# Owen1B/KAIR

Hardware: AMD Instinct MI355X
Metric: train patches/sec + PSNR, SwinIR x4 48-px LQ, at 1/2/4/8 MI355X (higher is better)
Workload: dtype fp32x3

## Files before the change

### kair_amd/csrc/gemm_x3.hip

```cpp
#include <string.h>

#include <type_traits>

#include "gemm_common.h"

namespace {

template <typename T> struct RawX3 { Raw<T> h, l; };

KAIR_DEV f32x4 mfma16(const f16x8& a, const f16x8& b, f32x4 c) {
  return __builtin_amdgcn_mfma_f32_16x16x32_f16(a, b, c, 0, 0, 0);
}

KAIR_DEV void commit_lo_plane(f16* dst, const Raw<f16>& raw, const Pend& pd) {
  f16x8 q = __builtin_bit_cast(f16x8, raw.a);
  if (pd.scale == 0.f) q = f16x8{};
  if (pd.ones >= 0) q[pd.ones] = (f16)0.f;
  *(f16x8*)dst = q;
}

template <typename T>
KAIR_DEV void commit_pair(f16* hi, f16* lo, const RawX3<T>& raw, const Pend& pd, float onev) {
  if constexpr (sizeof(T) == 4) {
    commit_chunk<f16, T>(hi, raw.h, pd, false, onev);
// ... 34 lines not shown
  const int n0 = tn * BN;
  const int tid = threadIdx.x, lane = tid & 63, wave = tid >> 6;
  const int wm = wave / WN, wn = wave % WN;
  const int KB = 2 * ((K + 63) / 64) * 64;

  RowState ra[PA], rb[PB];
#pragma unroll
  for (int p = 0; p < PA; ++p) {
    const int c = tid + p * NT;
    ra[p] = row_state<AM, TA>(A, c < CA ? m0 + c / CPR : A.M);
    ra[p].scale *= A.x3s;
  }
#pragma unroll
  for (int p = 0; p < PB; ++p) {
    const int c = tid + p * NT;
    rb[p] = row_state<AM_ROWS, f16>(B, c < CB ? (long)(n0 + c / CPR) : B.M);
  }
  RawX3<TA> va[PA];
  Raw<f16> vbh[PB], vbl[PB];
  Pend pa[PA], pb[PB], pbl[PB];
  auto gload = [&](int kt) {
    const int k0 = kt * BK;
#pragma unroll
    for (int p = 0; p < PA; ++p) {
      const int k = k0 + ((tid + p * NT) % CPR) * 8;
      issue_chunk<AM, TA>(A, ra[p], k, K, va[p].h, pa[p]);
      if constexpr (sizeof(TA) == 2) {
        Pend d;
        issue_chunk<AM, TA>(A, ra[p], k, K, va[p].l, d, A.lo_ptr);
      }
    }
    const int kb = (k0 >> 6) * 128 + (k0 & 63);
#pragma unroll
    for (int p = 0; p < PB; ++p) {
      const int k = kb + ((tid + p * NT) % CPR) * 8;
      issue_chunk<AM_ROWS, f16>(B, rb[p], k, KB, vbh[p], pb[p]);
      issue_chunk<AM_ROWS, f16>(B, rb[p], k + 64, KB, vbl[p], pbl[p]);
    }
  };
  auto sstore = [&](int st) {
    f16* s0 = lds + st * STAGE;
#pragma unroll
    for (int p = 0; p < PA; ++p) {
      const int c = tid + p * NT;
      if (c < CA) {
        const int o = (c / CPR) * LD + (c % CPR) * 8;
        commit_pair<TA>(s0 + o, s0 + PLANE + o, va[p], pa[p], 1.f);
      }
    }
#pragma unroll
    for (int p = 0; p < PB; ++p) {
      const int c = tid + p * NT;
      if (c < CB) {
        const int o = BM * LD + (c / CPR) * LD + (c % CPR) * 8;
        commit_chunk<f16, f16>(s0 + o, vbh[p], pb[p]);
        commit_chunk<f16, f16>(s0 + PLANE + o, vbl[p], pbl[p]);
      }
    }
  };

  f32x4 acc[RM][RN];
#pragma unroll
  for (int i = 0; i < RM; ++i)
#pragma unroll
    for (int j = 0; j < RN; ++j) acc[i][j] = f32x4{0.f, 0.f, 0.f, 0.f};

  const int fr = lane & 15, fq = lane >> 4;
  const int nk = (K + BK - 1) / BK;
  gload(0);
  sstore(0);
  __syncthreads();
  for (int kt = 0; kt < nk; ++kt) {
    const int st = kt & 1;
    if (kt + 1 < nk) gload(kt + 1);
    const f16* sAh = lds + st * STAGE;
    const f16* sBh = sAh + BM * LD;
    const f16* sAl = sAh + PLANE;
    const f16* sBl = sAl + BM * LD;
    f16x8 ah[RM], al[RM], bh[RN], bl[RN];
#pragma unroll
    for (int i = 0; i < RM; ++i) {
      const int o = (wm * TM + i * 16 + fr) * LD + fq * 8;
      ah[i] = *(const f16x8*)(sAh + o);
      al[i] = *(const f16x8*)(sAl + o);
    }
#pragma unroll
    for (int j = 0; j < RN; ++j) {
      const int o = (wn * TN + j * 16 + fr) * LD + fq * 8;
      bh[j] = *(const f16x8*)(sBh + o);
      bl[j] = *(const f16x8*)(sBl + o);
    }
#pragma unroll
    for (int i = 0; i < RM; ++i)
#pragma unroll
      for (int j = 0; j < RN; ++j) {
        acc[i][j] = mfma16(ah[i], bh[j], acc[i][j]);
        acc[i][j] = mfma16(ah[i], bl[j], acc[i][j]);
        acc[i][j] = mfma16(al[i], bh[j], acc[i][j]);
      }
    if (kt + 1 < nk) sstore(st ^ 1);
    __syncthreads();
  }
  float* et = (float*)smem;
#pragma unroll
  for (int i = 0; i < RM; ++i)
#pragma unroll
    for (int j = 0; j < RN; ++j)
#pragma unroll
      for (int r = 0; r < 4; ++r) et[(wm * TM + i * 16 + fq * 4 + r) * EPI_LD + wn * TN + j * 16 + fr] = acc[i][j][r];
  __syncthreads();
  constexpr int CH = BM * BN / 8;
  for (int c = tid; c < CH; c += NT) {
    const int row = c / (BN / 8), col = (c % (BN / 8)) * 8;
    float v[8];
    const float4 a = *(const float4*)(et + row * EPI_LD + col);
    const float4 b = *(const float4*)(et + row * EPI_LD + col + 4);
    v[0] = a.x; v[1] = a.y; v[2] = a.z; v[3] = a.w; v[4] = b.x; v[5] = b.y; v[6] = b.z; v[7] = b.w;
#pragma unroll
    for (int j = 0; j < 8; ++j) v[j] *= E.acc_scale;
    epi_chunk(E, m0 + row, n0 + col, v);
  }
}

template <typename TA, typename TB, int AMB, int BN, int BKo>
__global__ __launch_bounds__(NT, 2) void gemm_tn_x3_kernel(Op A, Op B, float* ws, long M, int N, int K, long rows_per_split,
                                                           int tilesK, float acc_scale) {
  constexpr int BMr = 32;
  constexpr int LDA = BN + 8, LDB = BKo + 8;
  constexpr int WN = 2, WK = 2;
  constexpr int TN_ = BN / WN, TK_ = BKo / WK;
  constexpr int RN = TN_ / 16, RK = TK_ / 16;
  constexpr int CPA = BN / 8, CPB = BKo / 8;
  constexpr int CA = BMr * CPA, CB = BMr * CPB;
  constexpr int PA = (CA + NT - 1) / NT, PB = (CB + NT - 1) / NT;
  constexpr int PL = BMr * (LDA + LDB);
  constexpr int STAGE = 2 * PL;
  __shared__ __attribute__((aligned(16))) f16 lds[2 * STAGE];

  const int tn = blockIdx.x / tilesK, tk = blockIdx.x - (blockIdx.x / tilesK) * tilesK;
  const int n0 = tn * BN, k0 = tk * BKo;
  const long mbeg = (long)blockIdx.y * rows_per_split;
  long mend = mbeg + rows_per_split;
  if (mend > M) mend = M;
  const int tid = threadIdx.x, lane = tid & 63, wave = tid >> 6;
  const int wn = wave / WK, wk = wave % WK;

  RawX3<TA> va[PA];
  RawX3<TB> vb[PB];
  Pend pa[PA], pb[PB];
  auto gload = [&](long mb) {
#pragma unroll
    for (int p = 0; p < PA; ++p) {
      const int c = tid + p * NT;
      if (c < CA) {
        const long m = mb + c / CPA;
        RowState r = row_state<AM_ROWS, TA>(A, m < mend ? m : A.M);
        r.scale *= A.x3s;
        issue_chunk<AM_ROWS, TA>(A, r, n0 + (c % CPA) * 8, N, va[p].h, pa[p]);
        if constexpr (sizeof(TA) == 2) {
          Pend d;
          issue_chunk<AM_ROWS, TA>(A, r, n0 + (c % CPA) * 8, N, va[p].l, d, A.lo_ptr);
        }
      }
    }
#pragma unroll
    for (int p = 0; p < PB; ++p) {
      const int c = tid + p * NT;
      if (c < CB) {
        const long m = mb + c / CPB;
        RowState r = row_state<AMB, TB>(B, m < mend ? m : B.M);
        r.scale *= B.x3s;
        issue_chunk<AMB, TB>(B, r, k0 + (c % CPB) * 8, K, vb[p].h, pb[p]);
        if constexpr (sizeof(TB) == 2) {
          Pend d;
          issue_chunk<AMB, TB>(B, r, k0 + (c % CPB) * 8, K, vb[p].l, d, B.lo_ptr);
        }
      }
    }
  };
  const float onea = ldexpf(1.f, A.x3_exp), oneb = ldexpf(1.f, B.x3_exp);
  auto sstore = [&](int st) {
    f16* sAh = lds + st * STAGE;
    f16* sBh = sAh + BMr * LDA;
#pragma unroll
    for (int p = 0; p < PA; ++p) {
      const int c = tid + p * NT;
      if (c < CA) {
        const int o = (c / CPA) * LDA + (c % CPA) * 8;
        commit_pair<TA>(sAh + o, sAh + PL + o, va[p], pa[p], onea);
      }
    }
#pragma unroll
    for (int p = 0; p < PB; ++p) {
      const int c = tid + p * NT;
      if (c < CB) {
        const int o = (c / CPB) * LDB + (c % CPB) * 8;
        commit_pair<TB>(sBh + o, sBh + PL + o, vb[p], pb[p], oneb);
      }
    }
  };

  f32x4 acc[RN][RK];
#pragma unroll
  for (int i = 0; i < RN; ++i)
#pragma unroll
    for (int j = 0; j < RK; ++j) acc[i][j] = f32x4{0.f, 0.f, 0.f, 0.f};

  const int nsteps = mbeg < mend ? (int)((mend - mbeg + BMr - 1) / BMr) : 0;
  if (nsteps > 0) {
    gload(mbeg);
    sstore(0);
    __syncthreads();
  }
  const int q = (lane & 15) >> 2, p4 = (lane & 3) * 4, g8 = (lane >> 4) * 8;
  for (int it = 0; it < nsteps; ++it) {
    const int st = it & 1;
    if (it + 1 < nsteps) gload(mbeg + (long)(it + 1) * BMr);
    const f16* sAh = lds + st * STAGE;
    const f16* sBh = sAh + BMr * LDA;
    const f16* sAl = sAh + PL;
    const f16* sBl = sBh + PL;
    f16x8 ah[RN], al[RN], bh[RK], bl[RK];
#pragma unroll
    for (int i = 0; i < RN; ++i) {
      const int o = (g8 + q) * LDA + wn * TN_ + i * 16 + p4;
      ah[i] = trfrag<f16>(sAh + o, LDA);
      al[i] = trfrag<f16>(sAl + o, LDA);
    }
#pragma unroll
    for (int j = 0; j < RK; ++j) {
      const int o = (g8 + q) * LDB + wk * TK_ + j * 16 + p4;
      bh[j] = trfrag<f16>(sBh + o, LDB);
      bl[j] = trfrag<f16>(sBl + o, LDB);
    }
#pragma unroll
    for (int i = 0; i < RN; ++i)
#pragma unroll
      for (int j = 0; j < RK; ++j) {
        acc[i][j] = mfma16(ah[i], bh[j], acc[i][j]);
        acc[i][j] = mfma16(ah[i], bl[j], acc[i][j]);
        acc[i][j] = mfma16(al[i], bh[j], acc[i][j]);
      }
    if (it + 1 < nsteps) sstore(st ^ 1);
    __syncthreads();
  }
  const int fr = lane & 15, fq = lane >> 4;
  float* P = ws + (long)blockIdx.y * N * K;
#pragma unroll
  for (int i = 0; i < RN; ++i)
#pragma unroll
    for (int j = 0; j < RK; ++j)
#pragma unroll
      for (int r = 0; r < 4; ++r) {
        const int n = n0 + wn * TN_ + i * 16 + fq * 4 + r;
        const int k = k0 + wk * TK_ + j * 16 + fr;
        if (n < N && k < K) P[(long)n * K + k] = acc[i][j][r] * acc_scale;
      }
}

constexpr int XR_BM = 128, XR_NB = 3, XR_ASTAGE = XR_BM * 128;
template <int BN> struct XR {
  static constexpr int BSTAGE = BN * 128, NA = BN <= 192 ? 5 : 4, LDS = NA * XR_ASTAGE + XR_NB * BSTAGE + BN * 4;
  static constexpr int RN = BN / 32;
  static constexpr int BI = BN / 64;
};

enum { XE_ROWS_F32 = 0, XE_ROWS_PAIR = 1, XE_QKV = 2, XE_PSHUF = 3, XE_PUNSHUF = 4 };

constexpr int XS_CTAS = 4, XS_IT = 64, XS_N = 5;
__device__ unsigned long long g_x3_stamps[XS_CTAS * 8 * XS_IT * XS_N];
KAIR_DEV unsigned long long x3_now() {
  unsigned long long t;
  asm volatile("s_memtime %0\n\ts_waitcnt lgkmcnt(0)" : "=s"(t)::"memory");
  return t;
}

enum { XA_NONE = 0, XA_GELU = 1, XA_GELU_X = 2, XA_LEAKY = 3 };
enum { XG_MUL = 4, XG_LEAKY = 2 };

template <typename TA, int AM, int EM, int EX, int ACT, int GK, int BN, int BM = XR_BM>
__global__ __launch_bounds__(512, 1) void gemm_nt_x3_ring(Op A, Op B, Epi E, int K, int tilesN, int tilesM, int m_base) {
  constexpr int NA = XR<BN>::NA, RN = XR<BN>::RN, NP = RN / 2, BI = XR<BN>::BI, BSTAGE = XR<BN>::BSTAGE, WC = BN / 2;
  constexpr int RI = BM / 64, ASTAGE = BM * 128;
  static_assert(RI == 1 || RI == 2, "64- or 128-row tiles");
  constexpr int XLDS = EX == EX_LNB ? (4 * 2 * 32 * 2 + 8) * 4 : 0;
  __shared__ __attribute__((aligned(16))) char smem[NA * ASTAGE + XR_NB * BSTAGE + BN * 4 + XLDS];
  char* const sA = smem;
  char* const sB = smem + NA * ASTAGE;
  float* const sBias = (float*)(sB + XR_NB * BSTAGE);
  const int tid = threadIdx.x, lane = tid & 63, wave = __builtin_amdgcn_readfirstlane(tid >> 6);
  const int grp = wave >> 2, wm = (wave >> 1) & 1, wn = wave & 1;
  const int fr = lane & 15, fq = lane >> 4, q8 = lane & 7;
  const int cta = xcd_remap(blockIdx.x, gridDim.x);
  const int nt = cta % tilesN, mstride = gridDim.x / tilesN, mt0 = cta / tilesN;
  if (mt0 >= tilesM) return;
  const int ntile = (tilesM - mt0 + mstride - 1) / mstride;
  const int nk = K / 32;
  const int total = ntile * nk;
  const int n0 = nt * BN;
  const f16* zero = (const f16*)g_kair_zero_line;

  constexpr bool SW = EM != XE_ROWS_F32;
  constexpr int CB = SW ? 4 : 16;
  int c8[NP], oc[NP];
  long colo[NP];
#pragma unroll
  for (int p = 0; p < NP; ++p) {
    const int n = SW ? n0 + wn * WC + (2 * p + (fq & 1)) * 16 + (fq >> 1) * 8 : n0 + wn * WC + 2 * p * 16 + 4 * fq;
    c8[p] = n;
    oc[p] = E.ones_col >= n + CB && E.ones_col < n + CB + 4 ? 4 + E.ones_col - n - CB
                                                            : (E.ones_col >= n && E.ones_col < n + 4 ? E.ones_col - n : -1);
    if constexpr (EM == XE_QKV) {
      const int pw = E.nh * E.hdp;
      const int part = fdiv(n, E.d_pw), rr = n - part * pw;
      const int h = fdiv(rr, E.d_hdp), d = rr - h * E.hdp;
      colo[p] = (long)part * E.M * pw + (long)h * E.tok * E.hdp + d;
    } else if constexpr (EM == XE_PSHUF) {
      const int nf = E.N / (E.r * E.r), sp = n / nf, c = n - sp * nf, i = sp / E.r, j = sp - i * E.r;
      colo[p] = ((long)i * E.psW * E.r + j) * E.ldo + c;
    } else {
      colo[p] = n;
    }
  }
  for (int i = tid; i < BN; i += 512) sBias[i] = E.bias && n0 + i < (EX == EX_LNB ? E.lnC : E.N) ? E.bias[n0 + i] : 0.f;
  if constexpr (EX == EX_LNB)
    if (tid < 8) ((int*)(sBias + BN + 4 * 2 * 32 * 2))[tid] = 0;
  const f16* bsrc[BI];
#pragma unroll
  for (int ii = 0; ii < BI; ++ii) {
    const int r = (wave * BI + ii) * 8 + (lane >> 3), u = q8 ^ (r & 7);
    bsrc[ii] = n0 + r < (int)B.M ? (const f16*)B.ptr + (long)(n0 + r) * B.ld + (u < 4 ? u * 8 : 64 + (u - 4) * 8) : nullptr;
  }
  long aoff[RI];
  int ay[RI], ax[RI], au[RI];
  bool aok[RI];
  auto load_rows = [&](int i) __attribute__((always_inline)) {
    const int mt = mt0 + i * mstride;
#pragma unroll
    for (int ii = 0; ii < RI; ++ii) {
      const int r = (wave * RI + ii) * 8 + (lane >> 3);
      const int m = m_base + mt * BM + r;
      au[ii] = q8 ^ (r & 7);
      aok[ii] = m < (int)A.M;
      const int mm = aok[ii] ? m : 0;
      if constexpr (AM == AM_ROWS) {
        aoff[ii] = (long)win_to_token32(mm, A.win) * A.ld;
      } else {
        const int hw = A.d_hw.d;
        const int b = fdiv(mm, A.d_hw), p = mm - b * hw;
        ay[ii] = fdiv(p, A.d_imW);
        ax[ii] = p - ay[ii] * A.imW;
        aoff[ii] = (long)b * (hw >> (2 * A.up_sh));
      }
    }
  };
  int at = 0, ak = 0, as_ = 0, bk = 0, bs = 0;
  int a_tap = 0, a_c0 = 0;
  const float* arow[RI];
#pragma unroll
  for (int ii = 0; ii < RI; ++ii) arow[ii] = nullptr;
  auto set_tap = [&]() __attribute__((always_inline)) {
    int dy = a_tap / 3 - 1, dx = a_tap - (a_tap / 3) * 3 - 1;
    if (A.flip) { dy = -dy; dx = -dx; }
#pragma unroll
    for (int ii = 0; ii < RI; ++ii) {
      const int y = ay[ii] + dy, x = ax[ii] + dx;
      arow[ii] = aok[ii] && y >= 0 && y < A.imH && x >= 0 && x < A.imW
                     ? (const float*)A.ptr + (aoff[ii] + (long)(y >> A.up_sh) * (A.imW >> A.up_sh) + (x >> A.up_sh)) * A.ld +
                           au[ii] * 4
                     : nullptr;
    }
  };
  auto issue_a = [&]() __attribute__((always_inline)) {
    if (ak == 0) {
      load_rows(at);
      if constexpr (AM == AM_IM2COL) {
        a_tap = 0;
        a_c0 = 0;
        set_tap();
      }
    }
    const int k0 = ak * 32;
    char* st = sA + as_ * ASTAGE;
#pragma unroll
    for (int ii = 0; ii < RI; ++ii) {
      const void* src = zero;
      if constexpr (sizeof(TA) == 2) {
        const f16* pl = (const f16*)(au[ii] < 4 ? A.ptr : A.lo_ptr);
        if (aok[ii]) src = pl + aoff[ii] + k0 + (au[ii] & 3) * 8;
      } else if constexpr (AM == AM_ROWS) {
        if (aok[ii]) src = (const float*)A.ptr + aoff[ii] + k0 + au[ii] * 4;
      } else {
        if (arow[ii]) src = arow[ii] + a_c0;
      }
      if (!KAIR_DBG(E.dbg & 36)) glds16(src, st + (wave * RI + ii) * 1024);
    }
    if constexpr (AM == AM_IM2COL) {
      a_c0 += 32;
      if (a_c0 == A.imC) {
        a_c0 = 0;
        if (++a_tap < 9) set_tap();
      }
    }
    if (++ak == nk) { ak = 0; ++at; }
    if (++as_ == NA) as_ = 0;
  };
  auto issue_b = [&]() __attribute__((always_inline)) {
    const int k0 = bk * 32, kb = (k0 >> 6) * 128 + (k0 & 63);
    char* st = sB + bs * BSTAGE;
#pragma unroll
    for (int ii = 0; ii < BI; ++ii)
      if (!KAIR_DBG(E.dbg & 20)) glds16(bsrc[ii] ? (const void*)(bsrc[ii] + kb) : (const void*)zero, st + (wave * BI + ii) * 1024);
    if (++bk == nk) bk = 0;
    if (++bs == XR_NB) bs = 0;
  };
  auto nA = [&](int u) __attribute__((always_inline)) { return u + NA - 1 >= 0 && u + NA - 1 < total ? RI : 0; };
  auto nB = [&](int u) __attribute__((always_inline)) { return u + XR_NB - 1 >= 0 && u + XR_NB - 1 < total ? BI : 0; };
  for (int u = -(NA - 1); u < 0; ++u) {
    if (nA(u)) issue_a();
    if (nB(u)) issue_b();
  }

  f32x4 acc[RI][RN];
#pragma unroll
  for (int i = 0; i < RI; ++i)
#pragma unroll
    for (int jn = 0; jn < RN; ++jn) acc[i][jn] = f32x4{0.f, 0.f, 0.f, 0.f};
  f16x8 ah[RI], al[RI], bh[RN], bl[RN];

  const float as = A.x3s;
  auto load_frags = [&](int sa, int sb) __attribute__((always_inline)) {
    if (KAIR_DBG(E.dbg & 64)) return;
    const char* stA = sA + sa * ASTAGE;
    const char* stB = sB + sb * BSTAGE;
#pragma unroll
    for (int i = 0; i < RI; ++i) {
      const int r = grp * (BM / 2) + wm * (BM / 4) + i * 16 + fr;
      const char* row = stA + r * 128;
      if constexpr (sizeof(TA) == 2) {
        ah[i] = *(const f16x8*)(row + ((fq ^ (r & 7)) << 4));
        al[i] = *(const f16x8*)(row + (((4 + fq) ^ (r & 7)) << 4));
      } else {
        const float4 x0 = *(const float4*)(row + (((2 * fq) ^ (r & 7)) << 4));
        const float4 x1 = *(const float4*)(row + (((2 * fq + 1) ^ (r & 7)) << 4));
        const float xv[8] = {x0.x, x0.y, x0.z, x0.w, x1.x, x1.y, x1.z, x1.w};
#pragma unroll
        for (int c = 0; c < 8; ++c) {
          const float w = xv[c] * as;
          ah[i][c] = (f16)w;
          al[i][c] = (f16)(w - (float)ah[i][c]);
        }
      }
    }
#pragma unroll
    for (int jn = 0; jn < RN; ++jn) {
      const int n = wn * WC + jn * 16 + fr;
      const char* row = stB + n * 128;
      bh[jn] = *(const f16x8*)(row + ((fq ^ (n & 7)) << 4));
      bl[jn] = *(const f16x8*)(row + (((4 + fq) ^ (n & 7)) << 4));
    }
  };
  auto mfma_chunk = [&]() __attribute__((always_inline)) {
    if (KAIR_DBG(E.dbg & 2)) return;
#pragma unroll
    for (int i = 0; i < RI; ++i)
#pragma unroll
      for (int jn = 0; jn < RN; ++jn) {
        acc[i][jn] = mfma16(bh[jn], ah[i], acc[i][jn]);
        acc[i][jn] = mfma16(bl[jn], ah[i], acc[i][jn]);
        acc[i][jn] = mfma16(bh[jn], al[i], acc[i][jn]);
      }
  };
  auto ln_epilogue = [&](int ct, const int (&rowv)[RI], const bool (&okm)[RI], int nvm) __attribute__((always_inline)) -> int {
    float* const xch = sBias + BN;
    volatile int* const flg = (volatile int*)(xch + 4 * 2 * 32 * 2);
    const int rw = grp * 2 + wm, C = E.lnC;
    const long slot0 = ((long)(m_base / BM + mt0 + ct * mstride) * 4 + rw) * RI;
    long tr[RI];
    float mu[RI], rsd[RI];
#pragma unroll
    for (int i = 0; i < RI; ++i) {
      tr[i] = okm[i] ? rowv[i] : 0;
      mu[i] = E.lnmu[tr[i]];
      rsd[i] = E.lnrs[tr[i]];
    }
    nvm += 2 * RI;
#pragma unroll
    for (int i = 0; i < RI; ++i) {
      const float* xr = E.lnx + tr[i] * E.lnldx;
      float xh[24];
#pragma unroll
      for (int p = 0; p < NP; ++p)
#pragma unroll
        for (int h = 0; h < 2; ++h) {
          const float4 q = *(const float4*)(xr + c8[p] + 16 * h);
          xh[p * 8 + h * 4 + 0] = q.x; xh[p * 8 + h * 4 + 1] = q.y;
          xh[p * 8 + h * 4 + 2] = q.z; xh[p * 8 + h * 4 + 3] = q.w;
        }
      nvm += 2 * NP;
      float s1 = 0.f, s2 = 0.f;
#pragma unroll
      for (int j = 0; j < 24; ++j) {
        const int p = j >> 3, h = (j >> 2) & 1, c4 = j & 3, cc = c8[p] + 16 * h + c4;
        const float v = acc[i][2 * p + h][c4] * E.acc_scale;
        xh[j] = cc < C ? (xh[j] - mu[i]) * rsd[i] : 0.f;
        const float gy = v * sBias[cc - n0];
        s1 += gy;
        s2 += gy * xh[j];
      }
      s1 += __shfl_xor(s1, 16);
      s1 += __shfl_xor(s1, 32);
      s2 += __shfl_xor(s2, 16);
      s2 += __shfl_xor(s2, 32);
      if (fq == 0) {
        xch[((rw * 2 + wn) * 32 + i * 16 + fr) * 2] = s1;
        xch[((rw * 2 + wn) * 32 + i * 16 + fr) * 2 + 1] = s2;
      }
      float* const pg = E.lnpart + (slot0 + i) * 2 * C;
#pragma unroll
      for (int p = 0; p < NP; ++p)
#pragma unroll
        for (int h = 0; h < 2; ++h) {
          float dg[4], db[4];
#pragma unroll
          for (int c4 = 0; c4 < 4; ++c4) {
            const float v = acc[i][2 * p + h][c4] * E.acc_scale;
            dg[c4] = row16_sum(v * xh[p * 8 + h * 4 + c4]);
            db[c4] = row16_sum(v);
          }
          const int c = c8[p] + 16 * h;
          if (fr == 0 && c < C) {
            *(float4*)(pg + c) = make_float4(dg[0], dg[1], dg[2], dg[3]);
            *(float4*)(pg + C + c) = make_float4(db[0], db[1], db[2], db[3]);
          }
          nvm += n0 + wn * WC + 32 * p + 16 * h < C ? 2 : 0;
        }
    }
    asm volatile("s_waitcnt lgkmcnt(0)" ::: "memory");
    if (lane == 0) flg[wave] = ct + 1;
    while (flg[wave ^ 1] != ct + 1) __builtin_amdgcn_s_sleep(1);
    asm volatile("" ::: "memory");
#pragma unroll
    for (int i = 0; i < RI; ++i) {
      const volatile float* a0 = xch + ((rw * 2 + 0) * 32 + i * 16 + fr) * 2;
      const volatile float* a1 = xch + ((rw * 2 + 1) * 32 + i * 16 + fr) * 2;
      const float S1 = (a0[0] + a1[0]) / (float)C, S2 = (a0[1] + a1[1]) / (float)C;
      float sc = E.cps;
      if (E.cprs) {
        sc *= E.cprs[fdiv((int)tr[i], E.d_cprps)];
        nvm += 1;
      }
      const long cr = E.cpo ? token_to_win(tr[i], E.cpwin) : 0;
      const float* xr = E.lnx + tr[i] * E.lnldx;
      float* const dr = (float*)E.out + tr[i] * E.ldo;
#pragma unroll
      for (int p = 0; p < NP; ++p)
#pragma unroll
        for (int h = 0; h < 2; ++h) {
          const int c = c8[p] + 16 * h;
          const float4 xq = *(const float4*)(xr + c), dq = *(const float4*)(dr + c);
          const float xa[4] = {xq.x, xq.y, xq.z, xq.w}, da[4] = {dq.x, dq.y, dq.z, dq.w};
          float o[4];
#pragma unroll
          for (int c4 = 0; c4 < 4; ++c4) {
            const int cc = c + c4;
            const float v = acc[i][2 * p + h][c4] * E.acc_scale;
            const float xhat = (xa[c4] - mu[i]) * rsd[i];
            o[c4] = da[c4] + (cc < C ? rsd[i] * (v * sBias[cc - n0] - S1 - xhat * S2) : 0.f);
          }
          if (okm[i]) {
            *(float4*)(dr + c) = make_float4(o[0], o[1], o[2], o[3]);
            if (E.cpo) {
              f16x4 hi, lo;
#pragma unroll
              for (int c4 = 0; c4 < 4; ++c4) {
                const float w = opaque(o[c4] * sc);
                hi[c4] = (f16)w;
                lo[c4] = (f16)(w - (float)hi[c4]);
              }
              *(f16x4*)((f16*)E.cpo + cr * E.cpld + c) = hi;
              *(f16x4*)((f16*)E.cplo + cr * E.cpld + c) = lo;
            }
          }
        }
      nvm += 4 * NP + (__ballot(okm[i]) != 0 ? 2 * NP * (E.cpo ? 3 : 1) : 0);
    }
#pragma unroll
    for (int i = 0; i < RI; ++i)
#pragma unroll
      for (int jn = 0; jn < RN; ++jn) acc[i][jn] = f32x4{0.f, 0.f, 0.f, 0.f};
    return nvm;
  };
  auto compute = [&](bool tile_end, int ct) __attribute__((always_inline)) -> int {
    if (!tile_end || KAIR_DBG(E.dbg & 1)) {
      mfma_chunk();
      return 0;
    }
    int nvm = 0;
    int rowv[RI];
    long roff[RI];
    bool okm[RI];
    const int m0 = m_base + (mt0 + ct * mstride) * BM + grp * (BM / 2) + wm * (BM / 4) + fr;
#pragma unroll
    for (int i = 0; i < RI; ++i) {
      const int m = m0 + i * 16;
      okm[i] = m < (int)E.M;
      const int mm = okm[i] ? m : 0;
      roff[i] = 0;
      if constexpr (EM == XE_QKV) {
        const int win = fdiv(mm, E.d_tok);
        rowv[i] = win * E.nh * E.tok + (mm - win * E.tok);
      } else if constexpr (EM == XE_PSHUF) {
        const int hw = E.psH * E.psW, b = mm / hw, pp = mm - b * hw, y = pp / E.psW, x = pp - y * E.psW;
        rowv[i] = mm;
        roff[i] = (((long)b * E.psH * E.r + (long)y * E.r) * ((long)E.psW * E.r) + (long)x * E.r) * E.ldo;
      } else if constexpr (EM == XE_PUNSHUF) {
        const int Wr = E.psW * E.r, HWr = E.psH * E.r * Wr, b = mm / HWr, pp = mm - b * HWr, Y = pp / Wr, X = pp - Y * Wr;
        const int y = Y / E.r, x = X / E.r;
        rowv[i] = mm;
        roff[i] = (((long)b * E.psH + y) * E.psW + x) * E.ldo + (long)((Y - y * E.r) * E.r + (X - x * E.r)) * E.N;
      } else {
        rowv[i] = win_to_token32(mm, E.win);
      }
    }
    mfma_chunk();
    if constexpr (EX == EX_LNB) return ln_epilogue(ct, rowv, okm, nvm);
    float4 ex[RI][NP][2];
    float rs[RI];
#pragma unroll
    for (int i = 0; i < RI; ++i) rs[i] = 1.f;
    if constexpr (EX != EX_NONE) {
#pragma unroll
      for (int i = 0; i < RI; ++i)
#pragma unroll
        for (int p = 0; p < NP; ++p) {
          const float* src = EX == EX_RESID ? E.resid + (long)rowv[i] * E.ldr : (const float*)E.gate + (long)rowv[i] * E.ldg;
          ex[i][p][0] = *(const float4*)(src + c8[p]);
          ex[i][p][1] = *(const float4*)(src + c8[p] + CB);
        }
      nvm += 2 * RI * NP;
    }
    if constexpr (EX == EX_RESID) {
      const bool hs = E.rowscale != nullptr;
#pragma unroll
      for (int i = 0; i < RI; ++i) {
        const float r = *(hs ? E.rowscale + fdiv(rowv[i], E.d_rps) : (const float*)g_kair_zero_line);
        rs[i] = hs ? r : 1.f;
      }
      nvm += RI;
    }
    const int nst = EM == XE_ROWS_F32 ? (E.pre ? 4 : 2) : (E.out_lo ? 2 : 1) + (EM == XE_ROWS_PAIR && E.pre ? 2 : 0);
#pragma unroll
    for (int i = 0; i < RI; ++i) nvm += __ballot(okm[i]) != 0 ? NP * nst : 0;
#pragma unroll
    for (int i = 0; i < RI; ++i)
#pragma unroll
      for (int p = 0; p < NP; ++p) {
        float v[8];
        const float4 b0 = *(const float4*)(sBias + c8[p] - n0), b1 = *(const float4*)(sBias + c8[p] + CB - n0);
        const float bv[8] = {b0.x, b0.y, b0.z, b0.w, b1.x, b1.y, b1.z, b1.w};
#pragma unroll
        for (int c = 0; c < 4; ++c) {
          if constexpr (SW) {
            const auto r = __builtin_amdgcn_permlane16_swap(__float_as_uint(acc[i][2 * p][c]),
                                                            __float_as_uint(acc[i][2 * p + 1][c]), false, false);
            v[c] = __uint_as_float(r[0]) * E.acc_scale + bv[c];
            v[4 + c] = __uint_as_float(r[1]) * E.acc_scale + bv[4 + c];
          } else {
            v[c] = acc[i][2 * p][c] * E.acc_scale + bv[c];
            v[4 + c] = acc[i][2 * p + 1][c] * E.acc_scale + bv[4 + c];
          }
        }
        const int n = c8[p];
        if constexpr (EM == XE_QKV) {
          if (okm[i]) store8_f16pair(E.out, E.out_lo, colo[p] + (long)rowv[i] * E.hdp, v, E.oscale);
        } else {
          float pre[8];
#pragma unroll
          for (int c = 0; c < 8; ++c) pre[c] = v[c];
          if constexpr (ACT == XA_GELU) {
#pragma unroll
            for (int c = 0; c < 8; c += 2) {
              f32x2 y2, d2;
              gelu_erf_pair2((f32x2){v[c], v[c + 1]}, y2, d2);
              v[c] = y2.x;
              v[c + 1] = y2.y;
              pre[c] = d2.x;
              pre[c + 1] = d2.y;
            }
          } else if constexpr (ACT == XA_GELU_X) {
#pragma unroll
            for (int c = 0; c < 8; c += 2) {
              const f32x2 x2 = {v[c], v[c + 1]};
              const f32x2 y2 = x2 * (0.5f * (1.0f + erf_f32x2(x2 * 0.70710678118654752f)));
              v[c] = y2.x;
              v[c + 1] = y2.y;
            }
          } else if constexpr (ACT == XA_LEAKY) {
#pragma unroll
            for (int c = 0; c < 8; ++c) v[c] = v[c] > 0.f ? v[c] : v[c] * E.slope;
          }
          if constexpr (EX != EX_NONE) {
            const float x8[8] = {ex[i][p][0].x, ex[i][p][0].y, ex[i][p][0].z, ex[i][p][0].w,
                                 ex[i][p][1].x, ex[i][p][1].y, ex[i][p][1].z, ex[i][p][1].w};
#pragma unroll
            for (int c = 0; c < 8; ++c) {
              if constexpr (EX == EX_RESID) v[c] = x8[c] + rs[i] * v[c];
              else if constexpr (GK == XG_MUL) v[c] *= x8[c];
              else v[c] *= (x8[c] > 0.f ? 1.f : E.slope);
            }
          }
#pragma unroll
          for (int c = 0; c < 8; ++c) v[c] = c == oc[p] ? 1.f : v[c];
          const long rr = rowv[i];
          const bool st = !KAIR_DBG(E.dbg & 128) || v[0] == 1.2345e-30f;
          if (okm[i] && st) {
            if constexpr (EM == XE_ROWS_PAIR) {
              store8_f16pair(E.out, E.out_lo, rr * E.ldo + n, v, E.oscale);
            } else {
              float* d = (float*)E.out + (EM == XE_PSHUF || EM == XE_PUNSHUF ? roff[i] + colo[p] : rr * E.ldo + n);
              *(float4*)d = make_float4(v[0], v[1], v[2], v[3]);
              *(float4*)(d + CB) = make_float4(v[4], v[5], v[6], v[7]);
            }
            if (E.pre) {
              float* d = (float*)E.pre + rr * E.ldp + n;
              *(float4*)d = make_float4(pre[0], pre[1], pre[2], pre[3]);
              *(float4*)(d + CB) = make_float4(pre[4], pre[5], pre[6], pre[7]);
            }
          }
        }
      }
#pragma unroll
    for (int i = 0; i < RI; ++i)
#pragma unroll
      for (int jn = 0; jn < RN; ++jn) acc[i][jn] = f32x4{0.f, 0.f, 0.f, 0.f};
    return nvm;
  };

  const bool stamping = KAIR_DBG(E.dbg & 8) && blockIdx.x < XS_CTAS;
  unsigned long long* stp = g_x3_stamps + ((long)blockIdx.x * 8 + wave) * XS_IT * XS_N;
  auto stamp = [&](int t, int k) __attribute__((always_inline)) {
    if (stamping && t < XS_IT) {
      const unsigned long long tt = x3_now();
      if (lane == 0) stp[t * XS_N + k] = tt;
    }
  };
  auto run = [&](auto G) __attribute__((always_inline)) {
    constexpr int g = decltype(G)::value;
    int kc = 0, ct = 0, ra = 0, rb = 0;
    int e1 = 0, e2 = 0;
    for (int t = 0; t <= total; ++t) {
      stamp(t, 0);
      if (t < total) {
        const int n = e2 + nA(t - 1) + nB(t - 1) + e1;
        if (n == RI + BI) {
          if constexpr (RI + BI == 5) asm volatile("s_waitcnt vmcnt(5)" ::: "memory");
          else if constexpr (RI + BI == 4) asm volatile("s_waitcnt vmcnt(4)" ::: "memory");
          else if constexpr (RI + BI == 3) asm volatile("s_waitcnt vmcnt(3)" ::: "memory");
          else asm volatile("s_waitcnt vmcnt(2)" ::: "memory");
        } else {
          vm_wait(n);
        }
      }
      stamp(t, 1);
      ring_barrier();
      if (nA(t)) issue_a();
      if (nB(t)) issue_b();
      stamp(t, 2);
      int e0 = 0;
      if constexpr (g == 0) {
        if (t < total) {
          load_frags(ra, rb);
          stamp(t, 3);
          e0 = compute(kc == nk - 1, ct);
          if (++kc == nk) { kc = 0; ++ct; }
        }
      } else {
        if (t >= 1) {
          e0 = compute(kc == nk - 1, ct);
          if (++kc == nk) { kc = 0; ++ct; }
        }
        stamp(t, 3);
        if (t < total) load_frags(ra, rb);
      }
      if (t < total) {
        if (++ra == NA) ra = 0;
        if (++rb == XR_NB) rb = 0;
      }
      stamp(t, 4);
      e2 = e1;
      e1 = e0;
    }
  };
  if (grp == 0) {
    run(std::integral_constant<int, 0>{});
  } else {
    __builtin_amdgcn_s_setprio(1);
    run(std::integral_constant<int, 1>{});
  }
}

constexpr int XT_RB = 32, XT_NS = 3;
constexpr int XT_PART = XT_RB * 192 * 4, XT_STAGE = 2 * XT_PART;
constexpr int XT_DMA = 6;
static_assert(XT_DMA * (XT_NS - 2) == 6, "the steady-state wait immediate in gemm_tn_x3_ring");
enum { BT_ROWS = 0, BT_TAP = 1 };

KAIR_DEV int xt_swz_pair(int r) { return ((r & 3) << 1) | (((r >> 3) & 1) << 3); }

template <int BT, bool PR>
KAIR_DEV void tn_x3_body(const Op& A, const Op& B, float* ws, int M, int N, int K, int tilesK, int tile, int split, int rps,
                         float acc_scale, char* smem) {
  static_assert(!PR || BT == BT_ROWS, "fp16-pair operands: row operands only");
  constexpr int ES = PR ? 2 : 4;
  const int tid = threadIdx.x, lane = tid & 63, wave = __builtin_amdgcn_readfirstlane(tid >> 6);
  const int wn = wave >> 2, wk = wave & 3;
  const int fr = lane & 15, fq = lane >> 4;
  const int n0 = (tile / tilesK) * 192, k0 = (tile % tilesK) * 192;
  const int mbeg = split * rps;
  const int mend = mbeg + rps < M ? mbeg + rps : M;
  const int nch = mbeg < mend ? (mend - mbeg + XT_RB - 1) / XT_RB : 0;
  const char* zero = (const char*)g_kair_zero_line;

  int dr[3], dcA[3], dcB[3], dy[3], dx[3];
  const char* baseA[3];
  const char* baseB[3];
#pragma unroll
  for (int ii = 0; ii < 3; ++ii) {
    const int s = (wave * 3 + ii) * 64 + lane;
    const int r = s / 48, q = s - r * 48;
    dr[ii] = r;
    dy[ii] = dx[ii] = 0;
    if constexpr (PR) {
      const int u = q ^ xt_swz_pair(r);
      const int pl = u >= 24 ? 1 : 0, col = (u - 24 * pl) * 8;
      dcA[ii] = n0 + col < N ? n0 + col : -1;
      dcB[ii] = k0 + col < K ? k0 + col : -1;
      baseA[ii] = (const char*)(pl ? A.lo_ptr : A.ptr);
      baseB[ii] = (const char*)(pl ? B.lo_ptr : B.ptr);
    } else {
      const int u = q ^ (((r >> 3) & 3) << 2);
      dcA[ii] = n0 + u * 4 < N ? n0 + u * 4 : -1;
      const int k = k0 + u * 4;
      baseA[ii] = (const char*)A.ptr;
      baseB[ii] = (const char*)B.ptr;
      if constexpr (BT == BT_TAP) {
        const int tap = k < K ? k / B.imC : 0;
        dcB[ii] = k < K ? k - tap * B.imC : -1;
        dy[ii] = tap / 3 - 1;
        dx[ii] = tap - (tap / 3) * 3 - 1;
      } else {
        dcB[ii] = k < K ? k : -1;
      }
    }
  }
  int lc = 0, ls = 0;
  const bool lin = A.win.ws == 0 && (BT == BT_TAP || B.win.ws == 0);
  const char* pa[3];
  const char* pb[3];
  int px[3], py[3];
#pragma unroll
  for (int ii = 0; ii < 3; ++ii) {
    const long m = mbeg + dr[ii];
    pa[ii] = baseA[ii] + (m * A.ld + (dcA[ii] >= 0 ? dcA[ii] : 0)) * ES;
    if constexpr (BT == BT_ROWS) {
      pb[ii] = baseB[ii] + (m * B.ld + (dcB[ii] >= 0 ? dcB[ii] : 0)) * ES;
      px[ii] = py[ii] = 0;
    } else {
      const int mm = m < M ? (int)m : 0;
      const int p = mm - fdiv(mm, B.d_hw) * B.d_hw.d;
      py[ii] = fdiv(p, B.d_imW);
      px[ii] = p - py[ii] * B.imW;
      pb[ii] = baseB[ii] + ((m + (long)dy[ii] * B.imW + dx[ii]) * B.ld + (dcB[ii] >= 0 ? dcB[ii] : 0)) * ES;
    }
  }
  auto issue_next = [&]() {
    char* st = smem + ls * XT_STAGE;
    const int m0 = mbeg + lc * XT_RB;
#pragma unroll
    for (int ii = 0; ii < 3; ++ii) {
      const int m = m0 + dr[ii];
      const bool ok = m < mend;
      const void* sa = zero;
      const void* sb = zero;
      if (lin) {
        if (ok && dcA[ii] >= 0) sa = pa[ii];
        if constexpr (BT == BT_ROWS) {
          if (ok && dcB[ii] >= 0) sb = pb[ii];
        } else {
          const int yy = py[ii] + dy[ii], xx = px[ii] + dx[ii];
          if (ok && dcB[ii] >= 0 && yy >= 0 && yy < B.imH && xx >= 0 && xx < B.imW) sb = pb[ii];
          px[ii] += XT_RB;
          while (px[ii] >= B.imW) {
            px[ii] -= B.imW;
            if (++py[ii] == B.imH) py[ii] = 0;
          }
        }
        pa[ii] += (long)XT_RB * A.ld * ES;
        pb[ii] += (long)XT_RB * B.ld * ES;
      } else {
        const int mm = ok ? m : 0;
        if (ok && dcA[ii] >= 0) sa = baseA[ii] + ((long)win_to_token32(mm, A.win) * A.ld + dcA[ii]) * ES;
        if constexpr (BT == BT_ROWS) {
          if (ok && dcB[ii] >= 0) sb = baseB[ii] + ((long)win_to_token32(mm, B.win) * B.ld + dcB[ii]) * ES;
        } else {
          const int hw = B.d_hw.d;
          const int b = fdiv(mm, B.d_hw), p = mm - b * hw;
          const int y = fdiv(p, B.d_imW), x = p - y * B.imW;
          const int yy = y + dy[ii], xx = x + dx[ii];
          if (ok && dcB[ii] >= 0 && yy >= 0 && yy < B.imH && xx >= 0 && xx < B.imW)
            sb = baseB[ii] + (((long)b * hw + (long)yy * B.imW + xx) * B.ld + dcB[ii]) * ES;
        }
      }
      glds16(sa, st + (wave * 3 + ii) * 1024);
      glds16(sb, st + XT_PART + (wave * 3 + ii) * 1024);
    }
    ++lc;
    if (++ls == XT_NS) ls = 0;
  };

#pragma unroll
  for (int j = 0; j < XT_NS - 1; ++j)
    if (lc < nch) issue_next();

  f32x4 acc[3][6];
#pragma unroll
  for (int i = 0; i < 3; ++i)
#pragma unroll
    for (int j = 0; j < 6; ++j) acc[i][j] = f32x4{0.f, 0.f, 0.f, 0.f};

  const float sa = A.x3s, sb = B.x3s;
  const int bones = !PR && B.ones_col >= 0 && !B.ones_in_data && B.ones_col >= k0 && B.ones_col < k0 + 192 ? B.ones_col - k0 : -1;
  auto frag = [&](const char* part, int c, float s, f16x8& hi, f16x8& lo) {
    const char* p = part + fq * 8 * 768 + ((((c >> 2) ^ (fq << 2))) << 4) + (c & 3) * 4;
#pragma unroll
    for (int j = 0; j < 8; ++j) {
      const float w = *(const float*)(p + j * 768) * s;
      hi[j] = (f16)w;
      lo[j] = (f16)(w - (float)hi[j]);
    }
  };
  const int q4 = (lane & 15) >> 2, p4 = (lane & 3) * 4;
  auto frag_tr = [&](const char* part, int pl, int cb) -> f16x8 {
    const int c = cb + p4, u = pl * 24 + (c >> 3), ob = (c & 7) * 2;
    const int r0 = fq * 8 + q4, r1 = r0 + 4;
    const char* a0 = part + r0 * 768 + ((u ^ xt_swz_pair(r0)) << 4) + ob;
    const char* a1 = part + r1 * 768 + ((u ^ xt_swz_pair(r1)) << 4) + ob;
    const short4v x = __builtin_amdgcn_ds_read_tr16_b64_v4i16((__attribute__((address_space(3))) short4v*)a0);
    const short4v y = __builtin_amdgcn_ds_read_tr16_b64_v4i16((__attribute__((address_space(3))) short4v*)a1);
    short __attribute__((ext_vector_type(8))) s8 = {x[0], x[1], x[2], x[3], y[0], y[1], y[2], y[3]};
    return __builtin_bit_cast(f16x8, s8);
  };
  int cs = 0;
  for (int j = 0; j < nch; ++j) {
    const int ahead = (nch - 1 - j) < (XT_NS - 2) ? (nch - 1 - j) : (XT_NS - 2);
    if (ahead == XT_NS - 2) asm volatile("s_waitcnt vmcnt(6)" ::: "memory");
    else vm_wait(XT_DMA * ahead);
    ring_barrier();
    if (lc < nch) issue_next();
    const char* st = smem + cs * XT_STAGE;
    f16x8 ah[6], al[6], bh[3], bl[3];
    if constexpr (PR) {
#pragma unroll
      for (int i = 0; i < 6; ++i) {
        ah[i] = frag_tr(st, 0, wn * 96 + i * 16);
        al[i] = frag_tr(st, 1, wn * 96 + i * 16);
      }
#pragma unroll
      for (int i = 0; i < 3; ++i) {
        bh[i] = frag_tr(st + XT_PART, 0, wk * 48 + i * 16);
        bl[i] = frag_tr(st + XT_PART, 1, wk * 48 + i * 16);
      }
    } else {
#pragma unroll
// ... 452 lines not shown
```

Measured before the change: 664.5.

## Issue epilogue residual/gate loads before final MFMA chunk and remap lanes for row-major stores

For f16-input row-mode GEMMs with a residual or gate epilogue, the residual/gate/rowscale global loads are now issued before the last MFMA chunk, so their latency overlaps with the matrix math. For the fp32 row-output case it also remaps each lane to a different row/column quad via ds_bpermute, so the epilogue loads and stores cover contiguous 16-float spans per row instead of scattered 4-float pieces. This costs extra cross-lane permutes and register pressure from holding the loaded values across the MFMA chunk.

```diff
diff --git a/kair_amd/csrc/gemm_x3.hip b/kair_amd/csrc/gemm_x3.hip
--- a/kair_amd/csrc/gemm_x3.hip
+++ b/kair_amd/csrc/gemm_x3.hip
@@ -360,11 +360,14 @@
 
   constexpr bool SW = EM != XE_ROWS_F32;
   constexpr int CB = SW ? 4 : 16;
+  constexpr bool LO = sizeof(TA) == 2 && AM == AM_ROWS && EM == XE_ROWS_F32 && EX != EX_NONE && EX != EX_LNB;
+  const int er = LO ? lane >> 2 : fr, eq = LO ? lane & 3 : fq;
+  const int bpa = 4 * (16 * eq + er);
   int c8[NP], oc[NP];
   long colo[NP];
 #pragma unroll
   for (int p = 0; p < NP; ++p) {
-    const int n = SW ? n0 + wn * WC + (2 * p + (fq & 1)) * 16 + (fq >> 1) * 8 : n0 + wn * WC + 2 * p * 16 + 4 * fq;
+    const int n = SW ? n0 + wn * WC + (2 * p + (fq & 1)) * 16 + (fq >> 1) * 8 : n0 + wn * WC + 2 * p * 16 + 4 * eq;
     c8[p] = n;
     oc[p] = E.ones_col >= n + CB && E.ones_col < n + CB + 4 ? 4 + E.ones_col - n - CB
                                                             : (E.ones_col >= n && E.ones_col < n + 4 ? E.ones_col - n : -1);
@@ -658,7 +661,7 @@
     int rowv[RI];
     long roff[RI];
     bool okm[RI];
-    const int m0 = m_base + (mt0 + ct * mstride) * BM + grp * (BM / 2) + wm * (BM / 4) + fr;
+    const int m0 = m_base + (mt0 + ct * mstride) * BM + grp * (BM / 2) + wm * (BM / 4) + er;
 #pragma unroll
     for (int i = 0; i < RI; ++i) {
       const int m = m0 + i * 16;
@@ -681,10 +684,11 @@
         rowv[i] = win_to_token32(mm, E.win);
       }
     }
-    mfma_chunk();
+    constexpr bool EARLY = sizeof(TA) == 2 && AM == AM_ROWS && EX != EX_NONE && EX != EX_LNB;
+    if constexpr (!EARLY) mfma_chunk();
     if constexpr (EX == EX_LNB) return ln_epilogue(ct, rowv, okm, nvm);
     float4 ex[RI][NP][2];
-    float rs[RI];
+    float rs[RI], rl[RI];
 #pragma unroll
     for (int i = 0; i < RI; ++i) rs[i] = 1.f;
     if constexpr (EX != EX_NONE) {
@@ -698,14 +702,28 @@
         }
       nvm += 2 * RI * NP;
     }
+    const bool hs = EX == EX_RESID && E.rowscale != nullptr;
     if constexpr (EX == EX_RESID) {
-      const bool hs = E.rowscale != nullptr;
+#pragma unroll
+      for (int i = 0; i < RI; ++i) rl[i] = *(hs ? E.rowscale + fdiv(rowv[i], E.d_rps) : (const float*)g_kair_zero_line);
+      nvm += RI;
+    }
+    if constexpr (EARLY) {
+      mfma_chunk();
+      asm volatile("" : "+v"(acc[RI - 1][RN - 1]));
 #pragma unroll
       for (int i = 0; i < RI; ++i) {
-        const float r = *(hs ? E.rowscale + fdiv(rowv[i], E.d_rps) : (const float*)g_kair_zero_line);
-        rs[i] = hs ? r : 1.f;
-      }
-      nvm += RI;
+        if constexpr (EX == EX_RESID) land(rl[i]);
+#pragma unroll
+        for (int p = 0; p < NP; ++p) {
+          land(ex[i][p][0]);
+          land(ex[i][p][1]);
+        }
+      }
+    }
+    if constexpr (EX == EX_RESID) {
+#pragma unroll
+      for (int i = 0; i < RI; ++i) rs[i] = hs ? rl[i] : 1.f;
     }
     const int nst = EM == XE_ROWS_F32 ? (E.pre ? 4 : 2) : (E.out_lo ? 2 : 1) + (EM == XE_ROWS_PAIR && E.pre ? 2 : 0);
 #pragma unroll
@@ -719,15 +737,18 @@
         const float bv[8] = {b0.x, b0.y, b0.z, b0.w, b1.x, b1.y, b1.z, b1.w};
 #pragma unroll
         for (int c = 0; c < 4; ++c) {
+          unsigned a0 = __float_as_uint(acc[i][2 * p][c]), a1 = __float_as_uint(acc[i][2 * p + 1][c]);
           if constexpr (SW) {
-            const auto r = __builtin_amdgcn_permlane16_swap(__float_as_uint(acc[i][2 * p][c]),
-                                                            __float_as_uint(acc[i][2 * p + 1][c]), false, false);
-            v[c] = __uint_as_float(r[0]) * E.acc_scale + bv[c];
-            v[4 + c] = __uint_as_float(r[1]) * E.acc_scale + bv[4 + c];
-          } else {
-            v[c] = acc[i][2 * p][c] * E.acc_scale + bv[c];
-            v[4 + c] = acc[i][2 * p + 1][c] * E.acc_scale + bv[4 + c];
+            const auto r = __builtin_amdgcn_permlane16_swap(a0, a1, false, false);
+            a0 = r[0];
+            a1 = r[1];
           }
+          if constexpr (LO) {
+            a0 = (unsigned)__builtin_amdgcn_ds_bpermute(bpa, (int)a0);
+            a1 = (unsigned)__builtin_amdgcn_ds_bpermute(bpa, (int)a1);
+          }
+          v[c] = __uint_as_float(a0) * E.acc_scale + bv[c];
+          v[4 + c] = __uint_as_float(a1) * E.acc_scale + bv[4 + c];
         }
         const int n = c8[p];
         if constexpr (EM == XE_QKV) {
```

Result: no change. 670.0, median of 6 (+0.8%).
